# kumar-shridhar/PyTorch-BayesianCNN

Hardware: AMD Instinct MI355X
Metric: MC-forward samples/sec, BayesianAlexNet CIFAR-10 bs=512 num_ens=10 (higher is better)
Workload: dtype f32; 1 GPU; BayesianAlexNet 3x32x32 -> 10, layer_type=bbb, softplus, bs=512, num_ens=10, forward only; global_batch=512, num_ens_total=10, parallelism=single, launch=hipGraph replay, 2 lane(s) x 4 steps per launch

## Files before the change

pytorch-bayesiancnn_amd/csrc/pconv_body.cuh:

```cuda
#pragma once
#include <hip/hip_runtime.h>
#include <stdint.h>

#include "bbb_common.cuh"
#include "pconv_args.h"

namespace pconv {

typedef float f32x16 __attribute__((ext_vector_type(16)));
typedef float f32x4 __attribute__((ext_vector_type(4)));

constexpr int kThreads = 256;
constexpr int BN = 64;
constexpr int BK = 32;
constexpr int LDW = BN + 1;
constexpr int KCH = 256;
constexpr int TPC = KCH / BK;

constexpr int kPlain = 0, kSplit = 1, kSeq = 2, kPool = 3;

__device__ __forceinline__ float agpr_read(float a) {
    float v;
    asm volatile("v_accvgpr_read_b32 %0, %1" : "=v"(v) : "a"(a));
    return v;
}
__device__ __forceinline__ void agpr_write(float& a, float v) { asm volatile("v_accvgpr_write_b32 %0, %1" : "=a"(a) : "v"(v)); }
template <int BM, bool LRT, bool ILV, int MODE = kPlain, bool TR = false>
__device__ __forceinline__ void pconv_item(const PConvArgs& p, const int64_t item, const int ks = 0) {
    constexpr bool SPLIT = MODE == kSplit;
    constexpr bool SEQ = MODE == kSeq;
    constexpr bool POOL = MODE == kPool;
    static_assert(!POOL || !LRT || BM == 64, "the pooled LRT form: 64-image tiles (one accumulator pair per wave)");
    static_assert(!TR || (MODE == kPlain && !LRT), "the transposed item: plain BBB form only");
    constexpr int LDX = BM + 4;
    constexpr int NT = (BM >= 128) ? 2 : 1;
    constexpr int MT = (BM == 256) ? 2 : 1;
    constexpr int WSETS = LRT ? 2 : 1;
    constexpr int XL = BM / 4;
    constexpr int XRPP = kThreads / XL;
    constexpr int XPASS = BK / XRPP;

    __shared__ __attribute__((aligned(16))) float Xs[1][BK * LDX];
    __shared__ float Ws[1][WSETS][BK * LDW];
    __shared__ int32_t kt_w[2][KCH];
    __shared__ int32_t kt_x[2][KCH];
    __shared__ float sbias[POOL ? BN : 1];
    __shared__ float sbias2[(POOL && LRT) ? BN : 1];

    int g, j;
    if (p.x_ds == 0 || (p.x_div > 1 && p.x_off == 0 && p.G % (p.x_div * p.Ntiles) == 0)) {
        const int gs = p.x_div > 1 ? p.x_div * p.Ntiles : p.G;
        const int64_t per_step = (int64_t)p.Mtiles * gs;
        const int step = (int)(item / per_step);
        const int64_t r = item - (int64_t)step * per_step;
        j = (int)(r / gs);
        g = step * gs + (int)(r - (int64_t)j * gs);
    } else {
        g = (int)(item / p.Mtiles);
        j = (int)(item - (int64_t)g * p.Mtiles);
    }
    const int e = g / p.Ntiles;
    const int ue = p.unit_off + e;
    const int ew = p.unit_div > 1 ? ue / p.unit_div : e;
    const int ex = p.x_div > 1 ? (e + p.x_off) / p.x_div : (p.x_mod > 0 ? ue % p.x_mod : e);
    const int n0 = (g - e * p.Ntiles) * BN;
    const int pix = j / p.nbt;
    const int b0 = (j - pix * p.nbt) * BM;
    const int Wq = POOL ? p.Wo / 2 : p.Wo;
    const int oh0 = pix / Wq, ow0 = pix - oh0 * Wq;
    int ihb, iwb, r_lo, q_lo, nq, nrq, Keff, ntiles;
    float inv_nrq, inv_nq;
    const float inv_cin = 1.0f / (float)p.Cin;
    auto set_pixel = [&](int oh, int ow) {
        if constexpr (POOL) {
            oh = __builtin_amdgcn_readfirstlane(oh);
            ow = __builtin_amdgcn_readfirstlane(ow);
        }
        if constexpr (TR) {
            ihb = oh - p.ph;
            iwb = ow - p.pw;
            int nr;
            tr_axis(ihb, p.dh, p.up_h, p.tstep_h, p.kh, p.H, r_lo, nr);
            tr_axis(iwb, p.dw, p.up_w, p.tstep_w, p.kw, p.W, q_lo, nq);
            nrq = nr * nq;
            Keff = p.Cin * nrq;
            ntiles = (Keff + BK - 1) / BK;
            inv_nrq = nrq > 0 ? 1.0f / (float)nrq : 0.0f;
            inv_nq = nq > 0 ? 1.0f / (float)nq : 0.0f;
            return;
        }
        ihb = oh * p.sh - p.ph;
        iwb = ow * p.sw - p.pw;
        r_lo = ihb < 0 ? (-ihb + p.dh - 1) / p.dh : 0;
        q_lo = iwb < 0 ? (-iwb + p.dw - 1) / p.dw : 0;
        int r_hi = (p.H - 1 - ihb) >= 0 ? (p.H - 1 - ihb) / p.dh + 1 : 0;
        int q_hi = (p.W - 1 - iwb) >= 0 ? (p.W - 1 - iwb) / p.dw + 1 : 0;
        r_hi = r_hi < p.kh ? r_hi : p.kh;
        q_hi = q_hi < p.kw ? q_hi : p.kw;
        const int nr = r_hi > r_lo ? r_hi - r_lo : 0;
        nq = q_hi > q_lo ? q_hi - q_lo : 0;
        nrq = nr * nq;
        Keff = p.Cin * nrq;
        ntiles = (Keff + BK - 1) / BK;
        inv_nrq = nrq > 0 ? 1.0f / (float)nrq : 0.0f;
        inv_nq = nq > 0 ? 1.0f / (float)nq : 0.0f;
    };
    set_pixel(POOL ? 2 * oh0 : oh0, POOL ? 2 * ow0 : ow0);

    const int tid = threadIdx.x;
    const int lane = tid & 63;
    const int wave = __builtin_amdgcn_readfirstlane(tid >> 6);
    const int wn = (BM >= 128) ? 0 : (wave >> 1) * 32;
    const int wm = (BM >= 128) ? wave * 32 * MT : (wave & 1) * 32;

    constexpr uint32_t kOOB = 0xFFFFFFF0u;
    constexpr uint32_t kWInv = 0x7FFFFFF0u;
    const uint32_t kXInv = p.x_inv;
    const int64_t w_elems = (int64_t)p.Cout * p.Kp;
    const int64_t x_elems = (int64_t)p.Cin * p.H * p.W * p.B;
    const __amdgpu_buffer_rsrc_t xrs = __builtin_amdgcn_make_buffer_rsrc(
        const_cast<float*>(p.x + (int64_t)ex * p.x_ds), 0, (int)(x_elems * 4), 0x00020000);
    const __amdgpu_buffer_rsrc_t wrs = __builtin_amdgcn_make_buffer_rsrc(
        const_cast<float*>(p.w + (int64_t)ew * p.w_ds), 0, (int)(w_elems * 4), 0x00020000);
    const __amdgpu_buffer_rsrc_t w2rs = __builtin_amdgcn_make_buffer_rsrc(
        const_cast<float*>(LRT ? p.w2 + (int64_t)ew * p.w_ds : p.w), 0, (int)(w_elems * 4), 0x00020000);

    const int wkl = tid & 31, wnl = tid >> 5;
    const int xb4 = (tid % XL) * 4, xkr = tid / XL;
    const uint32_t xcol = (uint32_t)(b0 + xb4) * 4u;
    uint32_t wrow[8];
#pragma unroll
    for (int ps = 0; ps < 8; ++ps) wrow[ps] = (uint32_t)(n0 + wnl + ps * 8) * (uint32_t)p.Kp * 4u;

    float wregA[WSETS][8];
    f32x4 xregA[XPASS];

    auto fill_chunk = [&](int chunk) {
        const int k = chunk * KCH + tid;
        uint32_t wo = kWInv, xo = kXInv;
        if (k < Keff) {
            int ci, rq;
            if (p.wtap) {
                rq = (int)((float)k * inv_cin);
                ci = k - rq * p.Cin;
                if (ci < 0) { --rq; ci += p.Cin; } else if (ci >= p.Cin) { ++rq; ci -= p.Cin; }
            } else {
                ci = (int)((float)k * inv_nrq);
                rq = k - ci * nrq;
                if (rq < 0) { --ci; rq += nrq; } else if (rq >= nrq) { ++ci; rq -= nrq; }
            }
            int rr = (int)((float)rq * inv_nq);
            int qq = rq - rr * nq;
            if (qq < 0) { --rr; qq += nq; } else if (qq >= nq) { ++rr; qq -= nq; }
            if constexpr (TR) {
                const int r = r_lo + rr * p.tstep_h, q = q_lo + qq * p.tstep_w;
                wo = (uint32_t)(ci * p.khkw + r * p.kw + q) * 4u;
                xo = (uint32_t)((ci * p.H + (ihb + r * p.dh) / p.up_h) * p.W + (iwb + q * p.dw) / p.up_w) * (uint32_t)p.B * 4u;
            } else {
                const int r = r_lo + rr, q = q_lo + qq;
                wo = (p.wtap ? (uint32_t)((r * p.kw + q) * p.Cin + ci) : (uint32_t)(ci * p.khkw + r * p.kw + q)) * 4u;
                xo = (uint32_t)((ci * p.H + ihb + r * p.dh) * p.W + iwb + q * p.dw) * (uint32_t)p.B * 4u;
            }
        }
        kt_w[chunk & 1][tid] = (int32_t)wo;
        kt_x[chunk & 1][tid] = (int32_t)xo;
    };

    constexpr int NLOADS = 8 + XPASS;
    uint32_t loff[NLOADS];
    auto load_addr = [&](int tile) {
        const int buf = (tile / TPC) & 1;
        const int kb = (tile % TPC) * BK;
        const uint32_t wob = (uint32_t)kt_w[buf][kb + wkl];
#pragma unroll
        for (int ps = 0; ps < 8; ++ps) loff[ps] = wrow[ps] + wob;
#pragma unroll
        for (int ps = 0; ps < XPASS; ++ps) loff[8 + ps] = (uint32_t)kt_x[buf][kb + xkr + ps * XRPP] + xcol;
    };
    auto load_one = [&](int i, float (&wreg)[WSETS][8], f32x4 (&xreg)[XPASS]) {
        if (i < XPASS) {
            xreg[i] = __builtin_bit_cast(f32x4, __builtin_amdgcn_raw_buffer_load_b128(xrs, loff[8 + i], 0, 0));
        } else {
            const int ps = i - XPASS;
            wreg[0][ps] = __builtin_bit_cast(float, __builtin_amdgcn_raw_buffer_load_b32(wrs, loff[ps], 0, 0));
            if (LRT) wreg[WSETS - 1][ps] = __builtin_bit_cast(float, __builtin_amdgcn_raw_buffer_load_b32(w2rs, loff[ps], 0, 0));
        }
    };
    auto load_tile = [&](int tile, float (&wreg)[WSETS][8], f32x4 (&xreg)[XPASS]) {
        load_addr(tile);
#pragma unroll
        for (int i = 0; i < NLOADS; ++i) load_one(i, wreg, xreg);
    };

    auto store_tile = [&](int, float (&wreg)[WSETS][8], f32x4 (&xreg)[XPASS]) {
        constexpr int buf = 0;
#pragma unroll
        for (int s = 0; s < WSETS; ++s)
#pragma unroll
            for (int ps = 0; ps < 8; ++ps) Ws[buf][s][wkl * LDW + wnl + ps * 8] = wreg[s][ps];
#pragma unroll
        for (int ps = 0; ps < XPASS; ++ps)
            *reinterpret_cast<f32x4*>(&Xs[buf][(xkr + ps * XRPP) * LDX + xb4]) = xreg[ps];
    };

    f32x16 acc[NT][MT];
    f32x16 accv[NT][MT];
    float tot[(SEQ || POOL) ? NT : 1][(SEQ || POOL) ? MT : 1][16];
    float totv[(SEQ && LRT) ? NT : 1][(SEQ && LRT) ? MT : 1][16];
#pragma unroll
    for (int t = 0; t < NT; ++t)
#pragma unroll
        for (int u = 0; u < MT; ++u)
#pragma unroll
            for (int r = 0; r < 16; ++r) {
                acc[t][u][r] = 0.0f; accv[t][u][r] = 0.0f;
                if constexpr (SEQ) { agpr_write(tot[t][u][r], 0.0f); if constexpr (LRT) agpr_write(totv[t][u][r], 0.0f); }
                if constexpr (POOL) agpr_write(tot[t][u][r], -__builtin_inff());
            }

    const int lrow = lane & 31, lk = lane >> 5;

    constexpr int PD = (BM >= 128) ? 2 : 4;
    auto mma_tile = [&](bool more) {
        float ra[PD + 1][NT], ra2[PD + 1][NT], rb[PD + 1][MT];
        auto fetch = [&](int kk, int slot) {
            const int krow = kk * 2 + lk;
#pragma unroll
            for (int mt = 0; mt < MT; ++mt) rb[slot][mt] = Xs[0][krow * LDX + wm + mt * 32 + lrow];
#pragma unroll
            for (int nt = 0; nt < NT; ++nt) {
                ra[slot][nt] = Ws[0][0][krow * LDW + wn + nt * 32 + lrow];
                if (LRT) ra2[slot][nt] = Ws[0][WSETS - 1][krow * LDW + wn + nt * 32 + lrow];
            }
        };
#pragma unroll
        for (int i = 0; i < PD; ++i) fetch(i, i);
#pragma unroll
        for (int kk = 0; kk < BK / 2; ++kk) {
            if (ILV && kk < NLOADS) {
                if (more) load_one(kk, wregA, xregA);
                __builtin_amdgcn_sched_barrier(0);
            }
            if (kk + PD < BK / 2) fetch(kk + PD, (kk + PD) % (PD + 1));
            const int s = kk % (PD + 1);
#pragma unroll
            for (int nt = 0; nt < NT; ++nt) {
#pragma unroll
                for (int mt = 0; mt < MT; ++mt)
                    acc[nt][mt] = __builtin_amdgcn_mfma_f32_32x32x2f32(ra[s][nt], rb[s][mt], acc[nt][mt], 0, 0, 0);
                if (LRT) {
#pragma unroll
                    for (int mt = 0; mt < MT; ++mt)
                        accv[nt][mt] = __builtin_amdgcn_mfma_f32_32x32x2f32(ra2[s][nt], rb[s][mt] * rb[s][mt], accv[nt][mt], 0, 0, 0);
                }
            }
            if (!ILV) __builtin_amdgcn_sched_barrier(0);
        }
    };

    if constexpr (POOL) {
        const __amdgpu_buffer_rsrc_t brs0 = __builtin_amdgcn_make_buffer_rsrc(
            const_cast<float*>(p.bias ? p.bias + (int64_t)ew * p.b_ds : p.w), 0, p.bias ? p.Cout * 4 : 0, 0x00020000);
        if (tid < BN) sbias[tid] = __builtin_bit_cast(float, __builtin_amdgcn_raw_buffer_load_b32(brs0, (uint32_t)(n0 + tid) * 4u, 0, 0));
        if constexpr (LRT) {
            const __amdgpu_buffer_rsrc_t brs2 = __builtin_amdgcn_make_buffer_rsrc(
                const_cast<float*>(p.bias2 ? p.bias2 + (int64_t)ew * p.b_ds : p.w), 0, p.bias2 ? p.Cout * 4 : 0, 0x00020000);
            if (tid < BN) sbias2[tid] = __builtin_bit_cast(float, __builtin_amdgcn_raw_buffer_load_b32(brs2, (uint32_t)(n0 + tid) * 4u, 0, 0));
        }
        __syncthreads();
    }
#pragma clang loop unroll(disable)
    for (int wp = 0; wp < (POOL ? 4 : 1); ++wp) {
    if (POOL && wp > 0) set_pixel(2 * oh0 + (wp >> 1), 2 * ow0 + (wp & 1));
    int t0 = 0, t1 = ntiles;
    if constexpr (SPLIT) {
        t0 = (int)((int64_t)ks * ntiles / p.ksplit);
        t1 = (int)((int64_t)(ks + 1) * ntiles / p.ksplit);
    }
    if (t1 > t0) {
        const int c0 = t0 / TPC;
        fill_chunk(c0);
        __syncthreads();
        load_tile(t0, wregA, xregA);
        if ((c0 + 1) * KCH < Keff) fill_chunk(c0 + 1);
        store_tile(0, wregA, xregA);
        __syncthreads();
        const int nranges = SEQ ? p.ksplit : 1;
        int t = t0;
#pragma clang loop unroll(disable)
        for (int sr = 0; sr < nranges; ++sr) {
            const int tr1 = SEQ ? (int)((int64_t)(sr + 1) * ntiles / p.ksplit) : t1;
#pragma clang loop unroll(disable)
            for (; t < tr1; ++t) {
                const bool more = (t + 1) < t1;
                if (more) {
                    if (ILV) load_addr(t + 1);
                    else     load_tile(t + 1, wregA, xregA);
                }
                if ((t % TPC) == 1 && t / TPC >= c0 + 1 && (t / TPC + 1) * KCH < Keff) fill_chunk(t / TPC + 1);
                mma_tile(more);
                __syncthreads();
                if (more) store_tile(0, wregA, xregA);
                __syncthreads();
            }
            if constexpr (SEQ) {
                if (sr + 1 < nranges) {
#pragma unroll
                    for (int nt = 0; nt < NT; ++nt)
#pragma unroll
                        for (int mt = 0; mt < MT; ++mt)
#pragma unroll
                            for (int r = 0; r < 16; ++r) {
                                agpr_write(tot[nt][mt][r], agpr_read(tot[nt][mt][r]) + acc[nt][mt][r]);
                                acc[nt][mt][r] = 0.0f;
                                if constexpr (LRT) {
                                    agpr_write(totv[nt][mt][r], agpr_read(totv[nt][mt][r]) + accv[nt][mt][r]);
                                    accv[nt][mt][r] = 0.0f;
                                }
                            }
                }
            }
        }
        if constexpr (SEQ) {
#pragma unroll
            for (int nt = 0; nt < NT; ++nt)
#pragma unroll
                for (int mt = 0; mt < MT; ++mt)
#pragma unroll
                    for (int r = 0; r < 16; ++r) {
                        acc[nt][mt][r] = agpr_read(tot[nt][mt][r]) + acc[nt][mt][r];
                        if constexpr (LRT) accv[nt][mt][r] = agpr_read(totv[nt][mt][r]) + accv[nt][mt][r];
                    }
        }
    }
    if constexpr (POOL && !LRT) {
#pragma unroll
        for (int nt = 0; nt < NT; ++nt)
#pragma unroll
            for (int r = 0; r < 16; ++r) {
                const float bn = sbias[wn + nt * 32 + (r & 3) + 8 * (r >> 2) + 4 * lk];
#pragma unroll
                for (int mt = 0; mt < MT; ++mt) {
                    const float v = bbb::apply_act(acc[nt][mt][r] + bn, p.act);
                    agpr_write(tot[nt][mt][r], bbb::max_nan(agpr_read(tot[nt][mt][r]), v));
                    acc[nt][mt][r] = 0.0f;
                }
            }
    }
    if constexpr (POOL && LRT) {
        const int pixc = (2 * oh0 + (wp >> 1)) * p.Wo + 2 * ow0 + (wp & 1);
        const int HoWoC = p.Ho * p.Wo;
#pragma unroll
        for (int mt = 0; mt < MT; ++mt) {
            const int b = b0 + wm + mt * 32 + lrow;
            const int bglob = b + p.b_off + (p.unit_div > 1 ? (ue % p.unit_div) * p.B : 0);
#pragma unroll
            for (int nt = 0; nt < NT; ++nt)
#pragma unroll
                for (int r = 0; r < 16; ++r) {
                    const int nl = wn + nt * 32 + (r & 3) + 8 * (r >> 2) + 4 * lk;
                    const int n = n0 + nl;
                    float v = acc[nt][mt][r] + sbias[nl];
                    const float var = 1e-16f + (accv[nt][mt][r] + sbias2[nl]);
                    if (p.sample) {
                        float z;
                        if (p.eps_ext) {
                            const bool in = (b < p.B) & (n < p.Cout);
                            z = in ? p.eps_ext[(int64_t)e * ((int64_t)p.Cout * HoWoC * p.B) + ((int64_t)n * HoWoC + pixc) * p.B + b] : 0.0f;
                        } else {
                            const uint64_t idx = (uint64_t)(((int64_t)bglob * p.Cout + n) * HoWoC + pixc);
                            float z4[4];
                            bbb::normal4(idx >> 2, p.stream_id, p.call0 + (p.call_dev ? *p.call_dev : 0u) + (uint32_t)ew, p.k0, p.k1, z4);
                            const int c = (int)(idx & 3);
                            z = c == 0 ? z4[0] : c == 1 ? z4[1] : c == 2 ? z4[2] : z4[3];
                        }
                        v = v + __builtin_amdgcn_sqrtf(var) * z;
                    }
                    v = bbb::apply_act(v, p.act);
                    agpr_write(tot[nt][mt][r], bbb::max_nan(agpr_read(tot[nt][mt][r]), v));
                    acc[nt][mt][r] = 0.0f;
                    accv[nt][mt][r] = 0.0f;
                    __builtin_amdgcn_sched_barrier(0);
                }
        }
    }
    }
    if constexpr (POOL) {
#pragma unroll
        for (int nt = 0; nt < NT; ++nt)
#pragma unroll
            for (int mt = 0; mt < MT; ++mt)
#pragma unroll
                for (int r = 0; r < 16; ++r) acc[nt][mt][r] = agpr_read(tot[nt][mt][r]);
    }

    if constexpr (SPLIT) {
        constexpr int TILE = 64 * BM;
        constexpr int TW = (BK * LDX) / 1024 >= 4 ? 4 : 2;
        __shared__ int s_last;
        const int S = p.ksplit;
        const __amdgpu_buffer_rsrc_t prs = __builtin_amdgcn_make_buffer_rsrc(
            p.part + (int64_t)item * S * (WSETS * TILE), 0, S * WSETS * TILE * 4, 0x00020000);
        float* const T = &Xs[0][(wave % TW) * 1024];
#pragma unroll
        for (int set = 0; set < WSETS; ++set)
#pragma unroll
            for (int nt = 0; nt < NT; ++nt)
#pragma unroll
                for (int mt = 0; mt < MT; ++mt)
#pragma unroll
                    for (int pass = 0; pass < 4 / TW; ++pass) {
                        if ((wave / TW) == pass) {
#pragma unroll
                            for (int r = 0; r < 16; ++r)
                                T[((r & 3) + 8 * (r >> 2) + 4 * lk) * 32 + lrow] = set == 0 ? acc[nt][mt][r] : accv[nt][mt][r];
#pragma unroll
                            for (int i = 0; i < 4; ++i) {
                                const int nl = (lane >> 3) + 8 * i, b4 = (lane & 7) * 4;
                                const f32x4 v4 = *reinterpret_cast<const f32x4*>(&T[nl * 32 + b4]);
                                const uint32_t off = (uint32_t)(((ks * WSETS + set) * 64 + wn + nt * 32 + nl) * BM + wm + mt * 32 + b4) * 4u;
                                __builtin_amdgcn_raw_buffer_store_b128(
                                    __builtin_bit_cast(__attribute__((__vector_size__(4 * sizeof(uint32_t)))) uint32_t, v4), prs, off, 0, 16);
                            }
                        }
                        if (TW < 4) __syncthreads();
                    }
        asm volatile("s_waitcnt vmcnt(0)" ::: "memory");
        __syncthreads();
        if (tid == 0) {
            const int old = __hip_atomic_fetch_add(p.tickets + item, 1, __ATOMIC_RELAXED, __HIP_MEMORY_SCOPE_AGENT);
            s_last = old == S - 1;
            if (old == S - 1) __hip_atomic_store(p.tickets + item, 0, __ATOMIC_RELAXED, __HIP_MEMORY_SCOPE_AGENT);
        }
        __syncthreads();
        if (!s_last) return;
        const int HoWo = p.Ho * p.Wo;
        const __amdgpu_buffer_rsrc_t yrs = __builtin_amdgcn_make_buffer_rsrc(
            p.y + (int64_t)e * p.y_ds, 0, (int)((int64_t)p.Cout * HoWo * p.B * 4), 0x00020000);
        const float* __restrict__ b1g = p.bias ? p.bias + (int64_t)ew * p.b_ds : nullptr;
        const float* __restrict__ b2g = (LRT && p.bias2) ? p.bias2 + (int64_t)ew * p.b_ds : nullptr;
#pragma unroll
        for (int q = 0; q < BM / 16; ++q) {
            const int f = q * kThreads + tid;
            const int nl = f / (BM / 4), b4 = (f % (BM / 4)) * 4;
            f32x4 sum[WSETS];
#pragma unroll
            for (int set = 0; set < WSETS; ++set) {
                sum[set] = __builtin_bit_cast(f32x4, __builtin_amdgcn_raw_buffer_load_b128(prs, (uint32_t)((set * 64 + nl) * BM + b4) * 4u, 0, 16));
                for (int k2 = 1; k2 < S; ++k2) {
                    const f32x4 v = __builtin_bit_cast(
                        f32x4, __builtin_amdgcn_raw_buffer_load_b128(prs, (uint32_t)(((k2 * WSETS + set) * 64 + nl) * BM + b4) * 4u, 0, 16));
#pragma unroll
                    for (int c = 0; c < 4; ++c) sum[set][c] += v[c];
                }
            }
            const int n = n0 + nl, bb = b0 + b4;
            if (n < p.Cout && bb < p.B) {
                const float bn = b1g ? b1g[n] : 0.0f;
                f32x4 o;
                if constexpr (!LRT) {
#pragma unroll
                    for (int c = 0; c < 4; ++c) o[c] = bbb::apply_act(sum[0][c] + bn, p.act);
                } else {
                    const float b2n = b2g ? b2g[n] : 0.0f;
                    const int64_t obase = (int64_t)e * p.y_ds + ((int64_t)n * HoWo + pix) * p.B + bb;
#pragma unroll
                    for (int c = 0; c < 4; ++c) {
                        float v = sum[0][c] + bn;
                        const float var = 1e-16f + (sum[WSETS - 1][c] + b2n);
                        if (p.y_mu) p.y_mu[obase + c] = v;
                        if (p.y_var) p.y_var[obase + c] = var;
                        if (p.sample) {
                            float z;
                            if (p.eps_ext) {
                                z = p.eps_ext[obase + c];
                            } else {
                                const int bglob = bb + c + p.b_off + (p.unit_div > 1 ? (ue % p.unit_div) * p.B : 0);
                                const uint64_t idx = (uint64_t)(((int64_t)bglob * p.Cout + n) * HoWo + pix);
                                float z4[4];
                                bbb::normal4(idx >> 2, p.stream_id, p.call0 + (p.call_dev ? *p.call_dev : 0u) + (uint32_t)ew, p.k0, p.k1, z4);
                                const int cc = (int)(idx & 3);
                                z = cc == 0 ? z4[0] : cc == 1 ? z4[1] : cc == 2 ? z4[2] : z4[3];
                            }
                            v = v + __builtin_amdgcn_sqrtf(var) * z;
                        }
                        o[c] = bbb::apply_act(v, p.act);
                    }
                }
                __builtin_amdgcn_raw_buffer_store_b128(__builtin_bit_cast(__attribute__((__vector_size__(4 * sizeof(uint32_t)))) uint32_t, o),
                                                       yrs, (uint32_t)(((int64_t)n * HoWo + pix) * p.B + bb) * 4u, 0, 0);
            }
        }
        return;
    }

    const int HoWo = POOL ? (p.Ho / 2) * (p.Wo / 2) : p.Ho * p.Wo;
    const __amdgpu_buffer_rsrc_t brs = __builtin_amdgcn_make_buffer_rsrc(
        const_cast<float*>(p.bias ? p.bias + (int64_t)ew * p.b_ds : p.w), 0, (p.bias && !POOL) ? p.Cout * 4 : 0, 0x00020000);
    const __amdgpu_buffer_rsrc_t yrs = __builtin_amdgcn_make_buffer_rsrc(
        p.y + (int64_t)e * p.y_ds, 0, (int)((int64_t)p.Cout * HoWo * p.B * 4), 0x00020000);
    if constexpr (!LRT || POOL) {
        constexpr int TW = (BK * LDX) / 1024 >= 4 ? 4 : 2;
        float* const T = &Xs[0][(wave % TW) * 1024];
#pragma unroll
        for (int mt = 0; mt < MT; ++mt)
#pragma unroll
            for (int nt = 0; nt < NT; ++nt) {
#pragma unroll
                for (int pass = 0; pass < 4 / TW; ++pass) {
                    if ((wave / TW) == pass) {
#pragma unroll
                        for (int r = 0; r < 16; ++r) T[((r & 3) + 8 * (r >> 2) + 4 * lk) * 32 + lrow] = acc[nt][mt][r];
#pragma unroll
                        for (int i = 0; i < 4; ++i) {
                            const int nl = (lane >> 3) + 8 * i, b4 = (lane & 7) * 4;
                            const int n = n0 + wn + nt * 32 + nl, bb = b0 + wm + mt * 32 + b4;
                            const float bn = __builtin_bit_cast(float, __builtin_amdgcn_raw_buffer_load_b32(brs, (uint32_t)n * 4u, 0, 0));
                            f32x4 v4 = *reinterpret_cast<const f32x4*>(&T[nl * 32 + b4]);
#pragma unroll
                            for (int c = 0; c < 4; ++c) v4[c] = POOL ? v4[c] : bbb::apply_act(v4[c] + bn, p.act);
                            const uint32_t off = ((bb < p.B) & (n < p.Cout)) ? (uint32_t)(((int64_t)n * HoWo + pix) * p.B + bb) * 4u : kOOB;
                            __builtin_amdgcn_raw_buffer_store_b128(
                                __builtin_bit_cast(__attribute__((__vector_size__(4 * sizeof(uint32_t)))) uint32_t, v4), yrs, off, 0, 0);
                        }
                    }
                    if (TW < 4) __syncthreads();
                }
            }
        return;
    }
    float bv[NT][16];
#pragma unroll
    for (int nt = 0; nt < NT; ++nt)
#pragma unroll
        for (int r = 0; r < 16; ++r) {
            const int n = n0 + wn + nt * 32 + (r & 3) + 8 * (r >> 2) + 4 * lk;
            bv[nt][r] = __builtin_bit_cast(float, __builtin_amdgcn_raw_buffer_load_b32(brs, (uint32_t)n * 4u, 0, 0));
        }
#pragma unroll
    for (int mt = 0; mt < MT; ++mt) {
        const int b = b0 + wm + mt * 32 + lrow;
        const bool b_ok = b < p.B;
        if (b_ok) {
            const int64_t ybase = (int64_t)e * p.y_ds + (int64_t)pix * p.B + b;
            const float* __restrict__ b2g = p.bias2 ? p.bias2 + (int64_t)ew * p.b_ds : nullptr;
            const int bglob = b + p.b_off + (p.unit_div > 1 ? (ue % p.unit_div) * p.B : 0);
#pragma unroll
            for (int nt = 0; nt < NT; ++nt) {
#pragma unroll
                for (int r = 0; r < 16; ++r) {
                    const int n = n0 + wn + nt * 32 + (r & 3) + 8 * (r >> 2) + 4 * lk;
                    if (n < p.Cout) {
                        const int64_t o = ybase + (int64_t)n * HoWo * p.B;
                        float v = acc[nt][mt][r] + bv[nt][r];
                        const float var = 1e-16f + (accv[nt][mt][r] + (b2g ? b2g[n] : 0.0f));
                        if (p.y_mu) p.y_mu[o] = v;
                        if (p.y_var) p.y_var[o] = var;
                        if (p.sample) {
                            float z;
                            if (p.eps_ext) {
                                z = p.eps_ext[o];
                            } else {
                                const uint64_t idx = (uint64_t)(((int64_t)bglob * p.Cout + n) * HoWo + pix);
                                float z4[4];
                                bbb::normal4(idx >> 2, p.stream_id, p.call0 + (p.call_dev ? *p.call_dev : 0u) + (uint32_t)ew, p.k0, p.k1, z4);
                                const int c = (int)(idx & 3);
                                z = c == 0 ? z4[0] : c == 1 ? z4[1] : c == 2 ? z4[2] : z4[3];
                            }
                            v = v + __builtin_amdgcn_sqrtf(var) * z;
                        }
                        p.y[o] = bbb::apply_act(v, p.act);
                    }
                }
            }
        }
    }
}

}
```

pytorch-bayesiancnn_amd/csrc/pconv_gemm.hip:

```cpp
#include <hip/hip_runtime.h>
#include <stdlib.h>
#include <stdint.h>

#include "../../include/bbb_hip.h"
#include "bbb_common.cuh"
#include "pconv_args.h"
#include "pconv_body.cuh"
#include "pconv_bf16x3.cuh"
#include "pconv_plan.h"

namespace {

using namespace pconv;

template <int BM, bool LRT, bool ILV, bool SEQ = false>
__global__ __launch_bounds__(kThreads) void pconv_gemm_kernel(const PConvArgs p) {
    const int bid = blockIdx.x;
    const int xcd = bid & 7;
    const int64_t item = (int64_t)xcd * p.per_xcd + (bid >> 3);
    const int64_t item_end = (int64_t)(xcd + 1) * p.per_xcd;
    if (item >= item_end || item >= (int64_t)p.G * p.Mtiles) return;
    pconv_item<BM, LRT, ILV, SEQ ? kSeq : kPlain>(p, item);
}

template <bool ILV>
__global__ __launch_bounds__(kThreads) __attribute__((amdgpu_waves_per_eu(4, 4))) void pconv_gemm_pool_kernel(const PConvArgs p) {
    const int bid = blockIdx.x;
    const int xcd = bid & 7;
    const int64_t item = (int64_t)xcd * p.per_xcd + (bid >> 3);
    const int64_t item_end = (int64_t)(xcd + 1) * p.per_xcd;
    if (item >= item_end || item >= (int64_t)p.G * p.Mtiles) return;
    pconv_item<128, false, ILV, kPool>(p, item);
}

__global__ __launch_bounds__(kThreads) void pconv_gemm_pool_lrt_kernel(const PConvArgs p) {
    const int bid = blockIdx.x;
    const int xcd = bid & 7;
    const int64_t item = (int64_t)xcd * p.per_xcd + (bid >> 3);
    const int64_t item_end = (int64_t)(xcd + 1) * p.per_xcd;
    if (item >= item_end || item >= (int64_t)p.G * p.Mtiles) return;
    pconv_item<64, true, false, kPool>(p, item);
}

template <int BM, bool LRT, bool ILV>
__global__ __launch_bounds__(kThreads) void pconv_gemm_splitk_kernel(const PConvArgs p) {
    const int bid = blockIdx.x;
    const int xcd = bid & 7;
    const int64_t blk = (int64_t)xcd * p.per_xcd + (bid >> 3);
    const int64_t blk_end = (int64_t)(xcd + 1) * p.per_xcd;
    if (blk >= blk_end || blk >= (int64_t)p.G * p.Mtiles * p.ksplit) return;
    const int64_t item = blk / p.ksplit;
    pconv_item<BM, LRT, ILV, kSplit>(p, item, (int)(blk - item * p.ksplit));
}

int fill(const bbb_conv_desc_t* d, PConvArgs& a) {
    pconv_plan::Geom g;
    const int rc = pconv_plan::describe(d, &g);
    if (rc != 0) return rc;
    a.x_inv = g.x_inv;
    a.B = g.B; a.Cin = g.Cin; a.H = g.H; a.W = g.W; a.Cout = g.Cout; a.kh = g.kh; a.kw = g.kw;
    a.sh = g.sh; a.sw = g.sw; a.ph = g.ph; a.pw = g.pw; a.dh = g.dh; a.dw = g.dw;
    a.Ho = g.Ho; a.Wo = g.Wo; a.K = g.K; a.khkw = g.khkw; a.act = g.act; a.Kp = g.Kp;
    a.x_ds = g.x_ds; a.w_ds = g.w_ds; a.b_ds = g.b_ds; a.y_ds = g.y_ds;
    a.unit_div = g.unit_div; a.unit_off = g.unit_off; a.x_mod = g.x_mod; a.b_off = g.b_off;
    a.x_div = g.x_div; a.x_off = g.x_off; a.pool = g.pool; a.wtap = g.wtap;
    return 0;
}

pconv_plan::Geom geom_of(const PConvArgs& a) {
    pconv_plan::Geom g = {};
    g.B = a.B; g.Cin = a.Cin; g.H = a.H; g.W = a.W; g.Cout = a.Cout; g.kh = a.kh; g.kw = a.kw;
    g.dh = a.dh; g.dw = a.dw; g.Ho = a.Ho; g.Wo = a.Wo; g.pool = a.pool;
    return g;
}

template <bool LRT>
int launch(PConvArgs& a, int draws, hipStream_t st) {
    using namespace pconv_plan;
    if (LRT && a.pool && (a.y_mu != nullptr || a.y_var != nullptr)) return BBB_EINVAL;
    Plan pl;
    const int rc = plan(geom_of(a), draws, LRT, a.ksplit, a.part != nullptr, &pl);
    if (rc != 0) return rc;
    a.Ntiles = pl.Ntiles; a.G = pl.G; a.nbt = pl.nbt; a.Mtiles = pl.Mtiles; a.per_xcd = pl.per_xcd;
    const dim3 grid((unsigned)pl.blocks), block(kThreads);
    if constexpr (LRT) {
        switch (pl.form) {
            case kLrtPool:  hipLaunchKernelGGL(pconv_gemm_pool_lrt_kernel, grid, block, 0, st, a); break;
            case kLrtCross: hipLaunchKernelGGL((pconv_gemm_splitk_kernel<64, true, true>), grid, block, 0, st, a); break;
            case kLrtSeq64: hipLaunchKernelGGL((pconv_gemm_kernel<64, true, false, true>), grid, block, 0, st, a); break;
            case kLrt64Ilv: hipLaunchKernelGGL((pconv_gemm_kernel<64, true, true>), grid, block, 0, st, a); break;
            case kLrt64:    hipLaunchKernelGGL((pconv_gemm_kernel<64, true, false>), grid, block, 0, st, a); break;
            default: return BBB_EINVAL;
        }
    } else {
        switch (pl.form) {
            case kBbbPool:      hipLaunchKernelGGL((pconv_gemm_pool_kernel<false>), grid, block, 0, st, a); break;
            case kBbbCross:     hipLaunchKernelGGL((pconv_gemm_splitk_kernel<64, false, true>), grid, block, 0, st, a); break;
            case kBbbSeq128Ilv: hipLaunchKernelGGL((pconv_gemm_kernel<128, false, true, true>), grid, block, 0, st, a); break;
            case kBbbSeq128:    hipLaunchKernelGGL((pconv_gemm_kernel<128, false, false, true>), grid, block, 0, st, a); break;
            case kBbbSeq64Ilv:  hipLaunchKernelGGL((pconv_gemm_kernel<64, false, true, true>), grid, block, 0, st, a); break;
            case kBbbSeq64:     hipLaunchKernelGGL((pconv_gemm_kernel<64, false, false, true>), grid, block, 0, st, a); break;
            case kBbb128Ilv:    hipLaunchKernelGGL((pconv_gemm_kernel<128, false, true>), grid, block, 0, st, a); break;
            case kBbb128:       hipLaunchKernelGGL((pconv_gemm_kernel<128, false, false>), grid, block, 0, st, a); break;
            case kBbb64Ilv:     hipLaunchKernelGGL((pconv_gemm_kernel<64, false, true>), grid, block, 0, st, a); break;
            case kBbb64:        hipLaunchKernelGGL((pconv_gemm_kernel<64, false, false>), grid, block, 0, st, a); break;
            default: return BBB_EINVAL;
        }
    }
    return (int)hipGetLastError();
}

}

namespace {
using pconv_plan::kTicketBytes;

int split_setup(PConvArgs& a, int draws, bool lrt, int k_split, void* scratch, int64_t scratch_bytes) {
    if (k_split <= 1) return 0;
    const pconv_plan::Geom g = geom_of(a);
    if (k_split != pconv_plan::canonical_ksplit(g)) return BBB_EINVAL;
    a.ksplit = k_split;
    const int64_t need = pconv_plan::split_scratch_bytes(g, draws, lrt, k_split);
    if (need > 0 && scratch != nullptr) {
        if (scratch_bytes < need || (((uintptr_t)scratch) & 255u) != 0) return BBB_EINVAL;
        a.tickets = static_cast<int32_t*>(scratch);
        a.part = reinterpret_cast<float*>(static_cast<char*>(scratch) + kTicketBytes);
    }
    return 0;
}
}

extern "C" int bbb_conv2d_chwn_plan(const bbb_conv_desc_t* d, int lrt, int k_split, int has_scratch, int32_t* form, int32_t* bm,
                                    int32_t* ilv, int64_t* items, int64_t* blocks) {
    pconv_plan::Geom g;
    int rc = pconv_plan::describe(d, &g);
    if (rc != 0) return rc;
    if (lrt && (d->w_draw_stride != 0 || d->b_draw_stride != 0)) return BBB_EINVAL;
    pconv_plan::Plan pl;
    if ((rc = pconv_plan::plan(g, d->draws, lrt != 0, k_split, has_scratch != 0, &pl)) != 0) return rc;
    if (form) *form = pl.form;
    if (bm) *bm = pl.bm;
    if (ilv) *ilv = pl.ilv;
    if (items) *items = pl.items;
    if (blocks) *blocks = pl.blocks;
    return 0;
}

extern "C" int64_t bbb_conv2d_chwn_splitk_scratch(const bbb_conv_desc_t* d, int lrt, int32_t* k_split) {
    PConvArgs a = {};
    if (k_split) *k_split = 1;
    if (fill(d, a) != 0) return 0;
    const pconv_plan::Geom g = geom_of(a);
    const int s = pconv_plan::canonical_ksplit(g);
    if (k_split) *k_split = s;
    return pconv_plan::split_scratch_bytes(g, d->draws, lrt != 0, s);
}

extern "C" int bbb_conv2d_chwn_splitk_fwd(const bbb_conv_desc_t* d, const float* x, const float* w, const float* bias, float* y,
                                          int k_split, void* scratch, int64_t scratch_bytes, void* stream) {
    PConvArgs a = {};
    int rc = fill(d, a);
    if (rc != 0) return rc;
    if (x == nullptr || w == nullptr || y == nullptr) return BBB_EINVAL;
    if ((((uintptr_t)x | (uintptr_t)y) & 15u) != 0 || (((uintptr_t)w | (uintptr_t)bias) & 3u) != 0) return BBB_EALIGN;
    a.x = x; a.w = w; a.bias = bias; a.y = y;
    if ((rc = split_setup(a, d->draws, false, k_split, scratch, scratch_bytes)) != 0) return rc;
    return launch<false>(a, d->draws, (hipStream_t)stream);
}

extern "C" int bbb_conv2d_chwn_fwd(const bbb_conv_desc_t* d, const float* x, const float* w, const float* bias, float* y,
                                   void* stream) {
    PConvArgs a = {};
    const int rc = fill(d, a);
    if (rc != 0) return rc;
    if (x == nullptr || w == nullptr || y == nullptr) return BBB_EINVAL;
    if ((((uintptr_t)x | (uintptr_t)y) & 15u) != 0 || (((uintptr_t)w | (uintptr_t)bias) & 3u) != 0) return BBB_EALIGN;
    a.x = x; a.w = w; a.bias = bias; a.y = y;
    return launch<false>(a, d->draws, (hipStream_t)stream);
}

extern "C" int bbb_conv2d_chwn_bf16x3_fwd(const bbb_conv_desc_t* d, const void* x, const float* w, const float* bias, void* y,
                                          uint32_t flags, void* stream) {
    PConvArgs a = {};
    const int rc = fill(d, a);
    if (rc != 0) return rc;
    if (x == nullptr || w == nullptr || y == nullptr || (flags & ~3u) != 0 || a.pool || a.wtap) return BBB_EINVAL;
    if ((((uintptr_t)x | (uintptr_t)y) & 15u) != 0 || (((uintptr_t)w | (uintptr_t)bias) & 3u) != 0) return BBB_EALIGN;
    const bool xs3 = (flags & BBB_S3_IN) != 0, ys3 = (flags & BBB_S3_OUT) != 0;
    if ((xs3 || ys3) && d->batch % 8 != 0) return BBB_ESHAPE;
    a.x = static_cast<const float*>(x); a.w = w; a.bias = bias; a.y = static_cast<float*>(y);
    a.x_ps = (int64_t)a.Cin * a.H * a.W * a.B;
    a.y_ps = (int64_t)a.Cout * a.Ho * a.Wo * a.B;
    if (ys3) a.y_ds = 3 * a.y_ps;
    if (xs3 && (d->x_draw_stride != 0 && d->x_draw_stride < 3 * a.x_ps)) return BBB_EINVAL;
    constexpr int kMT = 1;
    pconv_plan::Plan pl = {};
    if (const int rc = pconv_plan::channel_groups(a.Cout, d->draws, &pl)) return rc;
    if (const int rc = pconv_plan::item_grid(a.B, (int64_t)a.Ho * a.Wo, 128 * kMT, &pl)) return rc;
    a.Ntiles = pl.Ntiles; a.G = pl.G; a.nbt = pl.nbt; a.Mtiles = pl.Mtiles; a.per_xcd = pl.per_xcd;
    const dim3 grid((unsigned)pl.blocks), block(kThreads);
    hipStream_t st = (hipStream_t)stream;
    if (xs3 && ys3)      hipLaunchKernelGGL((pconv_bf16x3_kernel<kMT, true, true>), grid, block, 0, st, a);
    else if (xs3)        hipLaunchKernelGGL((pconv_bf16x3_kernel<kMT, true, false>), grid, block, 0, st, a);
    else if (ys3)        hipLaunchKernelGGL((pconv_bf16x3_kernel<kMT, false, true>), grid, block, 0, st, a);
    else                 hipLaunchKernelGGL((pconv_bf16x3_kernel<kMT, false, false>), grid, block, 0, st, a);
    return (int)hipGetLastError();
}

namespace {
typedef uint32_t s3_u32x4 __attribute__((ext_vector_type(4)));

__device__ __forceinline__ void s3_join(const s3_u32x4 h, const s3_u32x4 m, const s3_u32x4 l, float (&v)[8]) {
#pragma unroll
    for (int c = 0; c < 4; ++c) {
        v[2 * c] = (__builtin_bit_cast(float, h[c] << 16) + __builtin_bit_cast(float, m[c] << 16)) + __builtin_bit_cast(float, l[c] << 16);
        v[2 * c + 1] = (__builtin_bit_cast(float, h[c] & 0xFFFF0000u) + __builtin_bit_cast(float, m[c] & 0xFFFF0000u)) +
                       __builtin_bit_cast(float, l[c] & 0xFFFF0000u);
    }
}

__device__ __forceinline__ void s3_cut(const float (&v)[8], s3_u32x4& h, s3_u32x4& m, s3_u32x4& l) {
#pragma unroll
    for (int c = 0; c < 4; ++c) {
        uint32_t a0, a1, a2;
        split3_pair(f32x2{v[2 * c], v[2 * c + 1]}, a0, a1, a2);
        h[c] = a0; m[c] = a1; l[c] = a2;
    }
}

template <bool SQ>
__global__ __launch_bounds__(256) void maxpool_s3_kernel(const unsigned short* __restrict__ x, unsigned short* __restrict__ y,
                                                         int64_t total8, int C, int H, int W, int Ho, int Wo, int B8, int k, int s) {
    constexpr int NPL = SQ ? 6 : 3;
    const int64_t i = (int64_t)blockIdx.x * blockDim.x + threadIdx.x;
    if (i >= total8) return;
    const int b8 = (int)(i % B8);
    int64_t t = i / B8;
    const int ow = (int)(t % Wo);
    t /= Wo;
    const int oh = (int)(t % Ho);
    t /= Ho;
    const int c = (int)(t % C);
    const int64_t slab = t / C;
    const int64_t xps = (int64_t)C * H * W * B8, yps = (int64_t)C * Ho * Wo * B8;
    const s3_u32x4* xp = reinterpret_cast<const s3_u32x4*>(x) + slab * NPL * xps + (((int64_t)c * H + (int64_t)oh * s) * W + (int64_t)ow * s) * B8 + b8;
    float best[8];
    for (int a = 0; a < k; ++a)
        for (int q = 0; q < k; ++q) {
            const int64_t o = ((int64_t)a * W + q) * B8;
            float v[8];
            s3_join(xp[o], xp[o + xps], xp[o + 2 * xps], v);
#pragma unroll
            for (int u = 0; u < 8; ++u) best[u] = (a == 0 && q == 0) ? v[u] : bbb::max_nan(best[u], v[u]);
        }
    s3_u32x4 h, m, l;
    s3_cut(best, h, m, l);
    s3_u32x4* yp = reinterpret_cast<s3_u32x4*>(y) + slab * NPL * yps + (((int64_t)c * Ho + oh) * Wo + ow) * B8 + b8;
    yp[0] = h; yp[yps] = m; yp[2 * yps] = l;
    if constexpr (SQ) {
#pragma unroll
        for (int u = 0; u < 8; ++u) best[u] = bbb::mul_rn(best[u], best[u]);
        s3_cut(best, h, m, l);
        yp[3 * yps] = h; yp[4 * yps] = m; yp[5 * yps] = l;
    }
}

__global__ __launch_bounds__(256) void s3_from_f32_kernel(const float* __restrict__ x, unsigned short* __restrict__ y, int64_t n8, int64_t slabs) {
    const int64_t i = (int64_t)blockIdx.x * blockDim.x + threadIdx.x;
    if (i >= n8 * slabs) return;
    const int64_t slab = i / n8, j = i - slab * n8;
    const f32x4* xp = reinterpret_cast<const f32x4*>(x) + (slab * n8 + j) * 2;
    const f32x4 a = xp[0], b = xp[1];
    const float v[8] = {a[0], a[1], a[2], a[3], b[0], b[1], b[2], b[3]};
    s3_u32x4 h, m, l;
    s3_cut(v, h, m, l);
    s3_u32x4* yp = reinterpret_cast<s3_u32x4*>(y) + slab * 3 * n8 + j;
    yp[0] = h; yp[n8] = m; yp[2 * n8] = l;
}

__global__ __launch_bounds__(256) void s3_to_f32_kernel(const unsigned short* __restrict__ x, float* __restrict__ y, int64_t n8, int64_t slabs) {
    const int64_t i = (int64_t)blockIdx.x * blockDim.x + threadIdx.x;
    if (i >= n8 * slabs) return;
    const int64_t slab = i / n8, j = i - slab * n8;
    const s3_u32x4* xp = reinterpret_cast<const s3_u32x4*>(x) + slab * 3 * n8 + j;
    float v[8];
    s3_join(xp[0], xp[n8], xp[2 * n8], v);
    f32x4* yp = reinterpret_cast<f32x4*>(y) + (slab * n8 + j) * 2;
    yp[0] = f32x4{v[0], v[1], v[2], v[3]};
    yp[1] = f32x4{v[4], v[5], v[6], v[7]};
}
}

namespace {
int maxpool_s3_launch(const void* x, void* y, int64_t slabs, int channels, int h, int w, int batch, int k, int s, bool sq, void* stream) {
    if (x == nullptr || y == nullptr || slabs <= 0 || channels <= 0 || h <= 0 || w <= 0 || batch <= 0 || k <= 0 || s <= 0) return BBB_EINVAL;
    if (batch % 8 != 0 || h < k || w < k) return BBB_ESHAPE;
    if ((((uintptr_t)x | (uintptr_t)y) & 15u) != 0) return BBB_EALIGN;
    const int ho = (h - k) / s + 1, wo = (w - k) / s + 1;
    const int64_t total8 = slabs * channels * ho * wo * (batch / 8);
    const int64_t blocks = (total8 + 255) / 256;
    if (blocks > 0x7fffffffLL) return BBB_ESHAPE;
    if (sq) hipLaunchKernelGGL(maxpool_s3_kernel<true>, dim3((unsigned)blocks), dim3(256), 0, (hipStream_t)stream, static_cast<const unsigned short*>(x),
                               static_cast<unsigned short*>(y), total8, channels, h, w, ho, wo, batch / 8, k, s);
    else    hipLaunchKernelGGL(maxpool_s3_kernel<false>, dim3((unsigned)blocks), dim3(256), 0, (hipStream_t)stream, static_cast<const unsigned short*>(x),
                               static_cast<unsigned short*>(y), total8, channels, h, w, ho, wo, batch / 8, k, s);
    return (int)hipGetLastError();
}
}

extern "C" int bbb_maxpool_chwn_s3(const void* x, void* y, int64_t slabs, int channels, int h, int w, int batch, int k, int s, void* stream) {
    return maxpool_s3_launch(x, y, slabs, channels, h, w, batch, k, s, false, stream);
}

extern "C" int bbb_maxpool_chwn_s3sq(const void* x, void* y, int64_t slabs, int channels, int h, int w, int batch, int k, int s, void* stream) {
    return maxpool_s3_launch(x, y, slabs, channels, h, w, batch, k, s, true, stream);
}

extern "C" int bbb_s3_convert(const void* src, void* dst, int64_t slabs, int64_t n, int to_s3, void* stream) {
    if (src == nullptr || dst == nullptr || slabs <= 0 || n <= 0) return BBB_EINVAL;
    if (n % 8 != 0) return BBB_ESHAPE;
    if ((((uintptr_t)src | (uintptr_t)dst) & 15u) != 0) return BBB_EALIGN;
    const int64_t blocks = (slabs * (n / 8) + 255) / 256;
    if (blocks > 0x7fffffffLL) return BBB_ESHAPE;
    if (to_s3) hipLaunchKernelGGL(s3_from_f32_kernel, dim3((unsigned)blocks), dim3(256), 0, (hipStream_t)stream, static_cast<const float*>(src),
                                  static_cast<unsigned short*>(dst), n / 8, slabs);
    else       hipLaunchKernelGGL(s3_to_f32_kernel, dim3((unsigned)blocks), dim3(256), 0, (hipStream_t)stream,
                                  static_cast<const unsigned short*>(src), static_cast<float*>(dst), n / 8, slabs);
    return (int)hipGetLastError();
}

extern "C" int bbb_lrt_conv2d_chwn_splitk_fwd(const bbb_conv_desc_t* d, const float* x, const float* w_mu, const float* w_var,
                                              const float* b_mu, const float* b_var, float* y, float* act_mu_out,
                                              float* act_var_out, const float* eps_ext, uint64_t seed, uint32_t call0,
                                              uint32_t stream_id, int sample, const uint32_t* call_dev, int k_split,
                                              void* scratch, int64_t scratch_bytes, void* stream) {
// ... 27 lines not shown
```

Baseline: 7.862 million samples/s.

## Split each k-tile into half-stage load/store hand-over in 128-image conv GEMMs

Adds a HALF mode to the pconv item that splits each 32-deep k tile into two 16-deep halves. The next tile's global loads are issued and its shared-memory stores made per half, with a mid-tile barrier, so refilling the single LDS buffer overlaps the other half's MFMAs. The mode is enabled for the 128-image BBB plain/seq kernels (ILV or SEQ) and the pooled kernel. It also adds timestamp-probe macros (no-ops by default) and an experiment script to measure phase times. The extra barrier per tile and the changed weight-load mapping risk stalls or bank conflicts.

```diff
diff --git a/profiles/experiments/handover_stamps/run_stamps.py b/profiles/experiments/handover_stamps/run_stamps.py
--- /dev/null
+++ b/profiles/experiments/handover_stamps/run_stamps.py
@@ -0,0 +1,85 @@
+import ctypes
+import os
+import sys
+import time
+
+import numpy as np
+import torch
+
+HERE = os.path.dirname(os.path.abspath(__file__))
+ROOT = os.path.dirname(os.path.dirname(os.path.dirname(HERE)))
+sys.path.insert(0, os.path.join(ROOT, "pytorch-bayesiancnn_amd"))
+from bbb_hip.conv_desc import conv_desc, slab_rule
+
+PHASES = ["prologue", "phase A (k 0..5)", "wait at M", "phase B (k 6..15)", "wait at E", "epilogue"]
+B, STEPS, DRAWS = 512, 4, 10
+E = STEPS * DRAWS
+LAYERS = [("conv1 + pool1", 3, 32, 64, 11, 4, 5, True, True),
+          ("conv2", 64, 4, 192, 5, 1, 2, False, False),
+          ("conv4", 384, 2, 256, 3, 1, 1, False, False)]
+
+
+def main():
+    secs = float(sys.argv[1]) if len(sys.argv) > 1 else 2.0
+    lib = ctypes.CDLL(os.path.join(HERE, "libpconv_stamps.so"))
+    vp, i64 = ctypes.c_void_p, ctypes.c_int64
+    lib.pconv_stamps_set.argtypes = [vp, ctypes.c_ulonglong]
+    lib.bbb_conv2d_chwn_splitk_fwd.argtypes = [vp, vp, vp, vp, vp, ctypes.c_int, vp, i64, vp]
+    lib.bbb_conv2d_chwn_splitk_scratch.argtypes = [vp, ctypes.c_int, ctypes.POINTER(ctypes.c_int32)]
+    lib.bbb_conv2d_chwn_splitk_scratch.restype = i64
+    lib.bbb_conv2d_chwn_plan.argtypes = [vp, ctypes.c_int, ctypes.c_int, ctypes.c_int] + [vp] * 5
+    dev = torch.device("cuda:0")
+    stream = torch.cuda.current_stream().cuda_stream
+    print("# stamped half-stage hand-over: %d slabs, batch %d, %.1f s of back-to-back launches before the launch that is read" % (E, B, secs))
+    for name, cin, h, cout, k, s, p, pool, shared in LAYERS:
+        d, ho, wo = conv_desc(B, cin, (h, h), cout, (k, k), s, p, 1, act="softplus")
+        ex = STEPS if shared else E
+        slab_rule(d, ex, E, x_div=DRAWS if shared else 1)
+        d.pool = 1 if pool else 0
+        x = torch.randn(ex, cin, h, h, B, device=dev)
+        w = torch.randn(E, cout, cin, k, k, device=dev) * 0.05
+        b = torch.randn(E, cout, device=dev)
+        y = torch.empty(E, cout, ho // (2 if pool else 1), wo // (2 if pool else 1), B, device=dev)
+        ks = ctypes.c_int32(1)
+        lib.bbb_conv2d_chwn_splitk_scratch(ctypes.byref(d), 0, ctypes.byref(ks))
+        form, bm, ilv = ctypes.c_int32(), ctypes.c_int32(), ctypes.c_int32()
+        items, blocks = i64(), i64()
+        rc = lib.bbb_conv2d_chwn_plan(ctypes.byref(d), 0, ks.value, 0, ctypes.byref(form), ctypes.byref(bm), ctypes.byref(ilv),
+                                      ctypes.byref(items), ctypes.byref(blocks))
+        assert rc == 0, rc
+        nwaves = blocks.value * 4
+        stamps = torch.zeros(nwaves * 8, dtype=torch.int64, device=dev)
+        assert lib.pconv_stamps_set(stamps.data_ptr(), nwaves * 8) == 0
+
+        def launch():
+            rc = lib.bbb_conv2d_chwn_splitk_fwd(ctypes.byref(d), x.data_ptr(), w.data_ptr(), b.data_ptr(), y.data_ptr(), ks.value,
+                                                None, 0, stream)
+            assert rc == 0, rc
+
+        t0 = time.time()
+        n = 0
+        while time.time() - t0 < secs:
+            for _ in range(20):
+                launch()
+            torch.cuda.synchronize()
+            n += 20
+        stamps.zero_()
+        launch()
+        torch.cuda.synchronize()
+        assert lib.pconv_stamps_set(None, 0) == 0
+        a = stamps.cpu().numpy().reshape(-1, 4, 8).astype(np.float64)
+        a = a[a[:, :, 6].min(axis=1) > 0]
+        wg = a.mean(axis=1)
+        life = wg[:, :6].sum(axis=1)
+        tiles = wg[:, 6]
+        print("\n## %s: form %d, %d-image items, ilv %d, k_split %d, %d workgroups (%d stamped), %d warm launches"
+              % (name, form.value, bm.value, ilv.value, ks.value, blocks.value, len(a), n))
+        print("   k tiles per item: median %.0f (min %.0f, max %.0f); wave lifetime: median %.0f ticks" %
+              (np.median(tiles), tiles.min(), tiles.max(), np.median(life)))
+        print("   %-20s %12s %14s %8s" % ("phase", "ticks/item", "ticks/k tile", "share"))
+        for i, ph in enumerate(PHASES):
+            print("   %-20s %12.0f %14.2f %7.1f%%" % (ph, np.median(wg[:, i]), np.median(wg[:, i] / tiles), 100 * np.median(wg[:, i] / life)))
+
+
+if __name__ == "__main__":
+    main()
diff --git a/profiles/experiments/handover_stamps/stamps.hip b/profiles/experiments/handover_stamps/stamps.hip
--- /dev/null
+++ b/profiles/experiments/handover_stamps/stamps.hip
@@ -0,0 +1,32 @@
+#include <hip/hip_runtime.h>
+#include <stdint.h>
+
+namespace pconv_stamps {
+__device__ unsigned long long* buf = nullptr;
+__device__ unsigned long long cap = 0;
+}
+
+#define PCONV_STAMP_BEGIN() \
+    unsigned long long st_acc[8] = {}; \
+    unsigned long long st_last = __builtin_amdgcn_s_memtime(); \
+    st_acc[7] = st_last
+#define PCONV_STAMP(k) \
+    do { const unsigned long long st_now = __builtin_amdgcn_s_memtime(); st_acc[k] += st_now - st_last; st_last = st_now; } while (0)
+#define PCONV_STAMP_TILE() st_acc[6] += 1
+#define PCONV_STAMP_END() \
+    do { \
+        PCONV_STAMP(5); \
+        const unsigned long long st_i = ((unsigned long long)blockIdx.x * 4 + (threadIdx.x >> 6)) * 8; \
+        if ((threadIdx.x & 63) == 0 && pconv_stamps::buf != nullptr && st_i + 8 <= pconv_stamps::cap) { \
+            for (int st_k = 0; st_k < 8; ++st_k) pconv_stamps::buf[st_i + st_k] = st_acc[st_k]; \
+        } \
+    } while (0)
+
+#include "../../../pytorch-bayesiancnn_amd/csrc/pconv_gemm.hip"
+
+extern "C" int pconv_stamps_set(void* p, unsigned long long entries) {
+    unsigned long long* q = static_cast<unsigned long long*>(p);
+    if (hipMemcpyToSymbol(HIP_SYMBOL(pconv_stamps::buf), &q, sizeof(q)) != hipSuccess) return -1;
+    if (hipMemcpyToSymbol(HIP_SYMBOL(pconv_stamps::cap), &entries, sizeof(entries)) != hipSuccess) return -1;
+    return 0;
+}
diff --git a/pytorch-bayesiancnn_amd/csrc/pconv_body.cuh b/pytorch-bayesiancnn_amd/csrc/pconv_body.cuh
--- a/pytorch-bayesiancnn_amd/csrc/pconv_body.cuh
+++ b/pytorch-bayesiancnn_amd/csrc/pconv_body.cuh
@@ -4,6 +4,13 @@
 
 #include "bbb_common.cuh"
 #include "pconv_args.h"
+
+#ifndef PCONV_STAMP
+#define PCONV_STAMP_BEGIN()
+#define PCONV_STAMP(k)
+#define PCONV_STAMP_TILE()
+#define PCONV_STAMP_END()
+#endif
 
 namespace pconv {
 
@@ -25,9 +32,11 @@
     return v;
 }
 __device__ __forceinline__ void agpr_write(float& a, float v) { asm volatile("v_accvgpr_write_b32 %0, %1" : "=a"(a) : "v"(v)); }
-template <int BM, bool LRT, bool ILV, int MODE = kPlain, bool TR = false>
+template <int BM, bool LRT, bool ILV, int MODE = kPlain, bool TR = false, bool HALF = false>
 __device__ __forceinline__ void pconv_item(const PConvArgs& p, const int64_t item, const int ks = 0) {
     constexpr bool SPLIT = MODE == kSplit;
+    PCONV_STAMP_BEGIN();
+    static_assert(!HALF || (BM == 128 && !LRT && !TR && MODE != kSplit), "the half-stage hand-over: the 128-image BBB forms");
     constexpr bool SEQ = MODE == kSeq;
     constexpr bool POOL = MODE == kPool;
     static_assert(!POOL || !LRT || BM == 64, "the pooled LRT form: 64-image tiles (one accumulator pair per wave)");
@@ -125,12 +134,15 @@
     const __amdgpu_buffer_rsrc_t w2rs = __builtin_amdgcn_make_buffer_rsrc(
         const_cast<float*>(LRT ? p.w2 + (int64_t)ew * p.w_ds : p.w), 0, (int)(w_elems * 4), 0x00020000);
 
-    const int wkl = tid & 31, wnl = tid >> 5;
+    constexpr int WP = HALF ? 4 : 8;
+    constexpr int WSTEP = HALF ? 4 : 8;
+    const int wkl = HALF ? (tid & 15) : (tid & 31);
+    const int wnl = HALF ? ((tid >> 4) & 3) * 16 + (tid >> 6) : (tid >> 5);
     const int xb4 = (tid % XL) * 4, xkr = tid / XL;
     const uint32_t xcol = (uint32_t)(b0 + xb4) * 4u;
-    uint32_t wrow[8];
-#pragma unroll
-    for (int ps = 0; ps < 8; ++ps) wrow[ps] = (uint32_t)(n0 + wnl + ps * 8) * (uint32_t)p.Kp * 4u;
+    uint32_t wrow[WP];
+#pragma unroll
+    for (int ps = 0; ps < WP; ++ps) wrow[ps] = (uint32_t)(n0 + wnl + ps * WSTEP) * (uint32_t)p.Kp * 4u;
 
     float wregA[WSETS][8];
     f32x4 xregA[XPASS];
@@ -167,7 +179,38 @@
     };
 
     constexpr int NLOADS = 8 + XPASS;
-    uint32_t loff[NLOADS];
+    constexpr int HLOADS = 4 + XPASS / 2;
+    uint32_t loff[HALF ? HLOADS : NLOADS];
+    uint32_t htab[1 + XPASS / 2];
+    auto load_table_half = [&](int tile, int h) {
+        const int buf = (tile / TPC) & 1;
+        const int kb = (tile % TPC) * BK + h * (BK / 2);
+        htab[0] = (uint32_t)kt_w[buf][kb + wkl];
+#pragma unroll
+        for (int ps = 0; ps < XPASS / 2; ++ps) htab[1 + ps] = (uint32_t)kt_x[buf][kb + xkr + ps * XRPP];
+    };
+    auto load_addr_half = [&](bool more) {
+        const uint32_t wob = more ? htab[0] : kWInv;
+#pragma unroll
+        for (int ps = 0; ps < 4; ++ps) loff[ps] = wrow[ps % WP] + wob;
+#pragma unroll
+        for (int ps = 0; ps < XPASS / 2; ++ps) loff[4 + ps] = (more ? htab[1 + ps] : kXInv) + xcol;
+    };
+    auto load_one_half = [&](int h, int i) {
+        if (i < XPASS / 2) {
+            xregA[h * (XPASS / 2) + i] = __builtin_bit_cast(f32x4, __builtin_amdgcn_raw_buffer_load_b128(xrs, loff[4 + i], 0, 0));
+        } else {
+            const int ps = i - XPASS / 2;
+            wregA[0][h * 4 + ps] = __builtin_bit_cast(float, __builtin_amdgcn_raw_buffer_load_b32(wrs, loff[ps], 0, 0));
+        }
+    };
+    auto store_half = [&](int h) {
+#pragma unroll
+        for (int ps = 0; ps < 4; ++ps) Ws[0][0][(h * (BK / 2) + wkl) * LDW + wnl + ps * WSTEP] = wregA[0][h * 4 + ps];
+#pragma unroll
+        for (int ps = 0; ps < XPASS / 2; ++ps)
+            *reinterpret_cast<f32x4*>(&Xs[0][(h * (BK / 2) + xkr + ps * XRPP) * LDX + xb4]) = xregA[h * (XPASS / 2) + ps];
+    };
     auto load_addr = [&](int tile) {
         const int buf = (tile / TPC) & 1;
         const int kb = (tile % TPC) * BK;
@@ -255,6 +298,49 @@
                 }
             }
             if (!ILV) __builtin_amdgcn_sched_barrier(0);
+        }
+    };
+
+    constexpr int WK = 4;
+    auto mma_tile_half = [&](bool more, int tn) {
+        float ra[PD + 1][NT], rb[PD + 1][MT];
+        auto fetch = [&](int kk, int slot) {
+            const int krow = kk * 2 + lk;
+#pragma unroll
+            for (int mt = 0; mt < MT; ++mt) rb[slot][mt] = Xs[0][krow * LDX + wm + mt * 32 + lrow];
+#pragma unroll
+            for (int nt = 0; nt < NT; ++nt) ra[slot][nt] = Ws[0][0][krow * LDW + wn + nt * 32 + lrow];
+        };
+#pragma unroll
+        for (int i = 0; i < PD; ++i) fetch(i, i);
+#pragma unroll
+        for (int kk = 0; kk < BK / 2; ++kk) {
+            const int h = kk / (BK / 4), kh = kk % (BK / 4);
+            if (kh == 1) {
+                load_addr_half(more);
+                if (!ILV) {
+#pragma unroll
+                    for (int i = 0; i < HLOADS; ++i) load_one_half(h, i);
+                }
+            }
+            static_assert(HLOADS < BK / 4, "a half's loads are issued at k-steps 1..HLOADS of its phase");
+            if (ILV && kh >= 1 && kh <= HLOADS) load_one_half(h, kh - 1);
+            if (kh == WK) store_half(1 - h);
+            if (kk == BK / 4 - PD) {
+                PCONV_STAMP(1);
+                __syncthreads();
+                PCONV_STAMP(2);
+            }
+            __builtin_amdgcn_sched_barrier(0);
+            if (kk + PD < BK / 2) fetch(kk + PD, (kk + PD) % (PD + 1));
+            if (kh == 0) load_table_half(tn, h);
+            const int s = kk % (PD + 1);
+#pragma unroll
+            for (int nt = 0; nt < NT; ++nt)
+#pragma unroll
+                for (int mt = 0; mt < MT; ++mt)
+                    acc[nt][mt] = __builtin_amdgcn_mfma_f32_32x32x2f32(ra[s][nt], rb[s][mt], acc[nt][mt], 0, 0, 0);
+            __builtin_amdgcn_sched_barrier(0);
         }
     };
 
@@ -281,18 +367,40 @@
         const int c0 = t0 / TPC;
         fill_chunk(c0);
         __syncthreads();
-        load_tile(t0, wregA, xregA);
-        if ((c0 + 1) * KCH < Keff) fill_chunk(c0 + 1);
-        store_tile(0, wregA, xregA);
+        if constexpr (HALF) {
+#pragma unroll
+            for (int h = 0; h < 2; ++h) {
+                load_table_half(t0, h);
+                load_addr_half(true);
+#pragma unroll
+                for (int i = 0; i < HLOADS; ++i) load_one_half(h, i);
+            }
+            if ((c0 + 1) * KCH < Keff) fill_chunk(c0 + 1);
+            store_half(0);
+        } else {
+            load_tile(t0, wregA, xregA);
+            if ((c0 + 1) * KCH < Keff) fill_chunk(c0 + 1);
+            store_tile(0, wregA, xregA);
+        }
         __syncthreads();
         const int nranges = SEQ ? p.ksplit : 1;
         int t = t0;
+        PCONV_STAMP(0);
 #pragma clang loop unroll(disable)
         for (int sr = 0; sr < nranges; ++sr) {
             const int tr1 = SEQ ? (int)((int64_t)(sr + 1) * ntiles / p.ksplit) : t1;
 #pragma clang loop unroll(disable)
             for (; t < tr1; ++t) {
                 const bool more = (t + 1) < t1;
+                if constexpr (HALF) {
+                    if ((t % TPC) == 1 && t / TPC >= c0 + 1 && (t / TPC + 1) * KCH < Keff) fill_chunk(t / TPC + 1);
+                    mma_tile_half(more, t + 1);
+                    PCONV_STAMP(3);
+                    __syncthreads();
+                    PCONV_STAMP(4);
+                    PCONV_STAMP_TILE();
+                    continue;
+                }
                 if (more) {
                     if (ILV) load_addr(t + 1);
                     else     load_tile(t + 1, wregA, xregA);
@@ -527,6 +635,7 @@
                     if (TW < 4) __syncthreads();
                 }
             }
+        PCONV_STAMP_END();
         return;
     }
     float bv[NT][16];
diff --git a/pytorch-bayesiancnn_amd/csrc/pconv_gemm.hip b/pytorch-bayesiancnn_amd/csrc/pconv_gemm.hip
--- a/pytorch-bayesiancnn_amd/csrc/pconv_gemm.hip
+++ b/pytorch-bayesiancnn_amd/csrc/pconv_gemm.hip
@@ -12,6 +12,9 @@
 namespace {
 
 using namespace pconv;
+
+template <int BM, bool LRT, bool ILV, bool SEQ>
+constexpr bool kHalfStage = BM == 128 && !LRT && (ILV || SEQ);
 
 template <int BM, bool LRT, bool ILV, bool SEQ = false>
 __global__ __launch_bounds__(kThreads) void pconv_gemm_kernel(const PConvArgs p) {
@@ -20,7 +23,7 @@
     const int64_t item = (int64_t)xcd * p.per_xcd + (bid >> 3);
     const int64_t item_end = (int64_t)(xcd + 1) * p.per_xcd;
     if (item >= item_end || item >= (int64_t)p.G * p.Mtiles) return;
-    pconv_item<BM, LRT, ILV, SEQ ? kSeq : kPlain>(p, item);
+    pconv_item<BM, LRT, ILV, SEQ ? kSeq : kPlain, false, kHalfStage<BM, LRT, ILV, SEQ>>(p, item);
 }
 
 template <bool ILV>
@@ -30,7 +33,7 @@
     const int64_t item = (int64_t)xcd * p.per_xcd + (bid >> 3);
     const int64_t item_end = (int64_t)(xcd + 1) * p.per_xcd;
     if (item >= item_end || item >= (int64_t)p.G * p.Mtiles) return;
-    pconv_item<128, false, ILV, kPool>(p, item);
+    pconv_item<128, false, ILV, kPool, false, true>(p, item);
 }
 
 __global__ __launch_bounds__(kThreads) void pconv_gemm_pool_lrt_kernel(const PConvArgs p) {
```

Result: faster. 7.968 million samples/s (median of 6 runs) (+1.3%).
